# espnet/espnet

Hardware: AMD Instinct MI355X
Metric: audio-seconds/sec (RTF^-1), Conformer-ASR, 10 s utterances (higher is better)
Workload: dtype bf16; 1 GPU; BASELINE.json configs[1]: Conformer-small (12x256d, 4 heads), HIP STFT/log-mel + HIP encoder + greedy CTC (G1) + hypotheses collated to the host, 32 x 10 s utterances per GPU per step, V=5000; batch_per_gpu=32, global_batch=32, parallelism=utterance-dp1

## Files before the change

### espnet_amd/asr/encoder/conformer_encoder.py

```python
import ctypes as C
import math
import os
import threading
import weakref
from typing import List, Optional, Tuple

import torch

from espnet_amd import lib as L
from espnet_amd.nets_utils import (SUBSAMPLING_CONVS, SUBSAMPLING_MIN_FRAMES, conv2d_subsampled_lengths,
                                   conv_out_size)
from espnet_amd.packing import PackedModule

_POS_PROJ_LOCK = threading.Lock()
_ENC_CALL_LOCK = threading.Lock()
_TLS = threading.local()

LN_EPS = 1e-12


class LayerNorm(torch.nn.LayerNorm):
    def __init__(self, nout):
        super().__init__(nout, eps=LN_EPS)

# ... 58 lines not shown
        self.norm_ff_macaron = LayerNorm(size)
        self.norm_conv = LayerNorm(size)
        self.norm_final = LayerNorm(size)


def _fused_enabled(enc) -> bool:
    import os

    return bool(getattr(enc, "fused", True)) and os.environ.get("ESPNET_AMD_FUSED", "1") != "0"


def pack_k_units(w: torch.Tensor) -> torch.Tensor:
    n, k = w.shape
    assert k == 256 and n % 64 == 0, (n, k)
    return w.detach().reshape(n // 64, 4, 16, 8, 4, 8).permute(0, 1, 3, 4, 2, 5).contiguous().reshape(n, k)


def _pad_chunks(ff: int) -> int:
    assert ff % 64 == 0, ff
    return (ff + 127) // 128 * 128


def pack_w1(w: torch.Tensor) -> torch.Tensor:
    ff = w.shape[0]
    return pack_k_units(torch.nn.functional.pad(w.detach(), (0, 0, 0, _pad_chunks(ff) - ff)))


def pack_w2(w: torch.Tensor) -> torch.Tensor:
    d, ff = w.shape
    assert d == 256 and ff % 64 == 0, (d, ff)
# ... 209 lines not shown
                wqkv=A(torch.cat([sa.linear_q.weight, sa.linear_k.weight, sa.linear_v.weight], 0)),
                bqkv=F(torch.cat([sa.linear_q.bias, sa.linear_k.bias, sa.linear_v.bias], 0)),
                pos_u=F(sa.pos_bias_u), pos_v=F(sa.pos_bias_v),
                wout=A(sa.linear_out.weight), bout=F(sa.linear_out.bias),
                pw1=A(cm.pointwise_conv1.weight.reshape(2 * d, d)[glu_perm]),
                pw1_b=F(cm.pointwise_conv1.bias[glu_perm]),
                dw_w=F(dw_w.t()), dw_b=F(dw_b),
                pw2=A(cm.pointwise_conv2.weight.reshape(d, d)), pw2_b=F(cm.pointwise_conv2.bias),
                ff_w1=A(l.feed_forward.w_1.weight), ff_b1=F(l.feed_forward.w_1.bias),
                ff_w2=A(l.feed_forward.w_2.weight), ff_b2=F(l.feed_forward.w_2.bias),
            )
            pk.fill(layers[i], lt)
        if self._fusable():
            self._pack_fused(pk, layers)
            self._pack_fused_ctc(pk, w)
        elif self.em_dtype == L.EM_BF16 and d == 512 and ff % 128 == 0 and ff >= 256 and _fused_enabled(self):
            for i, l in enumerate(self.encoders):
                lt = dict(ffm_w1p=A(pack_ffn_rows_w1(l.feed_forward_macaron.w_1.weight)),
                          ffm_w2p=A(pack_ffn_rows_w2(l.feed_forward_macaron.w_2.weight)),
                          ff_w1p=A(pack_ffn_rows_w1(l.feed_forward.w_1.weight)),
                          ff_w2p=A(pack_ffn_rows_w2(l.feed_forward.w_2.weight)),
                          pw2p=A(pack_rows_proj(l.conv_module.pointwise_conv2.weight.reshape(d, d))),
                          woutp=A(pack_rows_proj(l.self_attn.linear_out.weight)),
                          pw1f=A(pack_rows_glu(l.conv_module.pointwise_conv1.weight.reshape(2 * d, d))),
                          fp_c=F(l.conv_module.pointwise_conv1.bias[glu_chunk_order(d)]))
                if self.heads * 64 == d:
                    sa = l.self_attn
                    lt["wqkvp"] = A(pack_ffn_rows_w1(torch.cat([sa.linear_q.weight, sa.linear_k.weight, sa.linear_v.weight], 0)))
                pk.fill(layers[i], lt)
            self._pack_rows_ctc(pk, w)
# ... 267 lines not shown
```

### espnet_amd/csrc/api.hip

```cpp
#include <stdlib.h>

#include <atomic>
#include <mutex>

#include "em_common.h"
#include "switches.h"

namespace {
EmSwitches read_switches() {
  auto on = [](const char* n) { return getenv(n) != nullptr; };
  auto num = [](const char* n, int dflt) { const char* e = getenv(n); return e ? atoi(e) : dflt; };
  EmSwitches s = {};
  s.attn2_stamps = on("EM_ATTN2_STAMPS"); s.block_stamps = on("EM_BLOCK_STAMPS"); s.ffn_stamps = on("EM_FFN_STAMPS");
  s.sub2_stamps = on("EM_SUB2_STAMPS");
  s.block_no_helpers = on("ESPNET_AMD_BLOCK_NO_HELPERS");
  s.sa_split = num("ESPNET_AMD_SA_SPLIT", 0); s.sa_group = num("ESPNET_AMD_SA_GROUP", 0);
  s.no_sa_tree = on("ESPNET_AMD_NO_SA_TREE"); s.sa_tree_min_rows = num("ESPNET_AMD_SA_TREE_MIN_ROWS", 200);
  s.no_attn2_large = on("ESPNET_AMD_NO_ATTN2_LARGE"); s.no_ffn_rows = on("ESPNET_AMD_NO_FFN_ROWS");
  s.no_rows_ctc = on("ESPNET_AMD_NO_ROWS_CTC"); s.frontend_v1 = on("ESPNET_AMD_FRONTEND_V1");
  s.gemm_stages = num("ESPNET_AMD_GEMM_STAGES", 0); s.gemm_bm = num("ESPNET_AMD_GEMM_BM", 0); s.no_mid_gemm = on("ESPNET_AMD_NO_MID_GEMM");
  s.mid_tile = num("ESPNET_AMD_MID_TILE", 0); s.lng_rt = num("ESPNET_AMD_LNG_RT", 0); s.lng_wide = num("ESPNET_AMD_LNG_WIDE", 256);
  s.no_src_lnq = on("ESPNET_AMD_NO_SRC_LNQ"); s.no_tail_fusion = on("ESPNET_AMD_NO_TAIL_FUSION");
  s.stream_no_fused = on("ESPNET_AMD_STREAM_NO_FUSED"); s.stream_mha_v1 = on("ESPNET_AMD_STREAM_MHA_V1");
  s.stream_no_ctx_fold = on("ESPNET_AMD_STREAM_NO_CTX_FOLD"); s.stream_no_ln_gemm = on("ESPNET_AMD_STREAM_NO_LN_GEMM");
  s.stream_fused_min = num("ESPNET_AMD_STREAM_FUSED_MIN", 1); s.no_sub12 = on("ESPNET_AMD_NO_SUB12");
  s.stream_ffn_split = num("ESPNET_AMD_STREAM_FFN_SPLIT", 0); s.stream_split_att = on("ESPNET_AMD_STREAM_SPLIT_ATT");
  s.dec_ffn_split = num("ESPNET_AMD_DEC_FFN_SPLIT", 0); s.dec_ffn_rows = num("ESPNET_AMD_DEC_FFN_ROWS", 0); s.no_rows_qkv = on("ESPNET_AMD_NO_ROWS_QKV"); s.ffn_rows_min_fill = num("ESPNET_AMD_FFN_ROWS_MIN_FILL", 0);
  return s;
}
std::atomic<const EmSwitches*> g_sw{nullptr};
std::mutex g_sw_mu;
}

const EmSwitches& em_sw() {
  const EmSwitches* p = g_sw.load(std::memory_order_acquire);
  if (!p) {
    std::lock_guard<std::mutex> lk(g_sw_mu);
    p = g_sw.load(std::memory_order_acquire);
    if (!p) {
      p = new EmSwitches(read_switches());
// ... 49 lines not shown
```

### espnet_amd/csrc/block.hip

```cpp
#include <stdio.h>
#include <stdlib.h>

#include <type_traits>

#include "em_common.h"
#include "switches.h"

namespace {

constexpr int D = 256;
constexpr int BM = 32;
constexpr int NT = 256;
constexpr int NC = 256;
constexpr int UNIT = 32768;
constexpr int PAR_FLOATS = EM_BLOCK_PARAM_GROUP;
constexpr int PAR_BYTES = PAR_FLOATS * 4;
constexpr int MAX_GROUPS = 4;
constexpr int PAR_OFF = 0;
constexpr int RED_OFF = PAR_OFF + MAX_GROUPS * PAR_BYTES;
constexpr int TOUCH_OFF = RED_OFF + 2048;
constexpr int TILE_OFF = TOUCH_OFF + 1024;
constexpr int ABUF_OFF = TILE_OFF + 32768;
constexpr int WK_OFF = ABUF_OFF + 16384;
constexpr int XCH_OFF = WK_OFF + 32768;
constexpr int XSLOT = 8192;
constexpr int SMEM_BYTES = XCH_OFF + 49152;
static_assert(ABUF_OFF % 1024 == 0 && TILE_OFF % 1024 == 0 && SMEM_BYTES <= 160 * 1024, "LDS layout");
constexpr int KW_MAX = 31, TROWS_MAX = BM + KW_MAX - 1;
constexpr int TPITCH = 528;
static_assert(TROWS_MAX * TPITCH <= 32768, "conv tile");
constexpr int CPAR_OFF = XCH_OFF;
constexpr int ABUF64_OFF = XCH_OFF + 8192;
static_assert(PAR_BYTES <= 8192 && ABUF64_OFF + 32768 <= SMEM_BYTES, "fold layout");

typedef const __attribute__((address_space(1))) unsigned char* GU8;
typedef const __attribute__((address_space(1))) bf16x8* GFRAG;
constexpr int BAR_UNIT = 1, BAR_PARAMS = 2, BAR_TILE = 4, BAR_LAST = 8;

#ifndef EM_BLOCK_DBG
#define EM_BLOCK_DBG 0
#endif

#ifndef EM_BLOCK_VAR
#define EM_BLOCK_VAR 0
#endif
#ifndef EM_BLOCK_FINE
#define EM_BLOCK_FINE 0
#endif
// ... 32 lines not shown
      if (ff_b1g) ff_b1g += sidx * nch_s * 64;
    }
  }
  bool ffn_exit = false;
  constexpr int KW = KWT, HALF = KWT / 2, TROWS = BM + KWT - 1;
  static_assert(KWT == 31 || KWT == 15, "depthwise conv width");
  constexpr int dbg = EM_BLOCK_DBG;
  using MM = Mma<bf16>;
  constexpr bool HAS_C = (MODE & EM_BLOCK_C) != 0, HAS_D = (MODE & EM_BLOCK_D) != 0;
  constexpr bool HAS_A = (MODE & EM_BLOCK_A) != 0, FINAL = (MODE & EM_BLOCK_FINAL) != 0;
  constexpr bool CTC = (MODE & EM_BLOCK_CTC) != 0;
  constexpr bool FOLD = HAS_C && HAS_D;
  constexpr bool ATT = (MODE & EM_BLOCK_ATT) != 0;
  static_assert(!ATT || (HAS_C && !HAS_D && !HAS_A && !FINAL), "block<ATT|C> is the only instantiation with the attention phase");
  static_assert(!FOLD || KWT == 31, "the folded C part is written for the 15-frame halo of k = 31");
  extern __shared__ __attribute__((aligned(1024))) unsigned char smem[];
  unsigned char* const abuf = smem + ABUF_OFF;
  float* const red0 = (float*)(smem + RED_OFF);
  float* const par = (float*)(smem + PAR_OFF);

  const int tid = threadIdx.x, lane = tid & 63;
  const int wave = __builtin_amdgcn_readfirstlane(tid >> 6);
  const int nf = wave & 3;
  const int lr = lane & 15, lg = lane >> 4;
  int b = blockIdx.y, t0 = blockIdx.x * BM;
  const int T = a.T;
  if constexpr (ATT) {
    const int gx = gridDim.x, lid = blockIdx.y * gx + blockIdx.x, grp = lid / (8 * gx);
    if ((int)blockIdx.y < a.B && grp * 8 + 8 <= a.B) {
      b = grp * 8 + (lid & 7);
// ... 196 lines not shown
    }
  };
  constexpr int MAXT = 16;
  auto touch = [&]() __attribute__((always_inline)) {
#ifdef EM_BLOCK_NO_TOUCH
    return;
#endif
    const int nwg = gridDim.x * gridDim.y;
    const int per_xcc = (nwg + 7) >> 3;
    const int nworker = per_xcc * 4;
    const int worker = (int)((blockIdx.y * gridDim.x + blockIdx.x) >> 3) * 4 + wave;
    const unsigned dst = TOUCH_OFF + wave * 256;
    const int loff = lane * 128;
    int total = (HAS_C ? 48 : 0) + (HAS_D ? 16 + 8 * nch : 0) + (HAS_A ? 48 + 8 * nch : 0);
    if (CTC) total += a.ctc_units * 4;
#pragma unroll 1
    for (int i = 0; i < MAXT && worker + i * nworker < total; ++i) {
      int j = worker + i * nworker;
      const unsigned char* p = nullptr;
      auto take = [&](const void* base, int n) __attribute__((always_inline)) {
        if (p == nullptr) {
          if (j < n) p = (const unsigned char*)base + (size_t)j * 8192;
          else j -= n;
        }
      };
      if (HAS_C) {
        take(a.wout, 16);
        take(a.pw1f, 32);
      }
      if (HAS_D) {
        take(a.pw2, 16);
        take(ff_w1, nch * 4);
        take(ff_w2, nch * 4);
      }
      if (HAS_A) {
        take(ffm_w1, nch * 4);
        take(ffm_w2, nch * 4);
        take(a.wqkv, 48);
      }
      if (CTC) take(a.ctc_w, a.ctc_units * 4);
// ... 1119 lines not shown
    }
    if constexpr (!HAS_A && !FINAL) {
      store_x();
      if (a.last_dst) {
        float* const dst = a.last_dst + (size_t)b * a.row_stride;
#pragma unroll
        for (int mi = 0; mi < 2; ++mi)
          if (t0 + mi * 16 + lr == T - 1) {
#pragma unroll
            for (int f = 0; f < 4; ++f) *(float4*)(dst + 64 * f + ncol) = xr[mi][f];
          }
      }
      touch_done();
      return;
    }
  } else {
    const bool ctx_slot = a.row0_src != nullptr && t0 == 0 && lr == 0;
    const float* const s0 = ctx_slot ? a.row0_src + (size_t)b * a.row_stride : a.x + mrow[0] * D;
#pragma unroll
    for (int f = 0; f < 4; ++f) xr[0][f] = *(const float4*)(s0 + 64 * f + ncol);
#pragma unroll
    for (int f = 0; f < 4; ++f) xr[1][f] = *(const float4*)(a.x + mrow[1] * D + 64 * f + ncol);
  }

  if (HAS_A) {
    stamp(30);
    const float* const pa0 = HAS_D ? pb2 : pb0;
    const float* const pa1 = HAS_D ? pb3 : pb1;
    if constexpr (HAS_D) {
      ln_to_act(pa0, 0, 256, 0);
    } else {
      touch();
      ln_to_act_pre(pa0, 0, 256, 0,
                    [&] { read_unit(ffm_w1, 0, ring[0]); read_unit(ffm_w1, 1, ring[1]); read_w2(ffm_w2, 0, 0, ring[2]); }, std::integral_constant<int, 24>{},
                    [&] { read_w2(ffm_w2, 0, 1, ring[3]); }, std::integral_constant<int, 8>{});
    }
    stamp(15);
    ffn(pa0, 512, 1536, 0.5f, ffm_w1, ffm_w2, true, ffm_b1g, a.wqkv, [&] { read_unit(a.wqkv, 2, ring[2]); });
    if constexpr (RELU) {
      if (ffn_exit) return;
    }
    stamp(22);
    ln_to_act(pa1, 0, 256, 0);
    stamp(15);
    const int H = D / 64;
    stream_k(a.wqkv, std::integral_constant<int, 12>{}, [&](const WF& cur, int u) {
      const int which = u >> 2, head = u & 3;
// ... 126 lines not shown
extern "C" int em_conformer_block_fused(int mode, const EmBlockArgs* a, void* stream) {
  if (!a || !a->x || !a->params || a->B <= 0 || a->T <= 0) return EM_ERR_BAD_ARG;
  const bool relu = (mode & EM_BLOCK_RELU) != 0;
  mode &= ~EM_BLOCK_RELU;
  if (a->d != D || a->ff <= 0 || a->ff % 64 != 0 || a->ff > 4096) return EM_ERR_UNSUPPORTED;
  hipStream_t s = (hipStream_t)stream;
  const bool need_a = (mode & EM_BLOCK_A) != 0, need_d = (mode & EM_BLOCK_D) != 0;
  if (!relu && a->ff > 1024 && (need_a || need_d)) return EM_ERR_UNSUPPORTED;
  if (relu && ((need_a && !a->ffm_b1g) || (need_d && !a->ff_b1g))) return EM_ERR_BAD_ARG;
  if (relu && mode != EM_BLOCK_A && mode != EM_BLOCK_D && mode != (EM_BLOCK_ATT | EM_BLOCK_C)) return EM_ERR_UNSUPPORTED;
  if (a->ffn_split > 1 && (need_a || need_d)) {
    const int nch_all = ((a->ff >> 6) + 1) & ~1;
    if (!relu || a->ffn_split > 16 || nch_all % (2 * a->ffn_split) != 0 || !a->ffn_part || !a->ffn_ticket) return EM_ERR_BAD_ARG;
  }
  if (!relu && mode == EM_BLOCK_D) return EM_ERR_UNSUPPORTED;
  if (need_a) {
    if (!a->ffm_w1 || !a->ffm_w2 || !a->wqkv || !a->qh || !a->kh || !a->vt) return EM_ERR_BAD_ARG;
    if (a->Tpad % 64 != 0 || a->Tpad < em_cdiv(a->T, BM) * BM) return EM_ERR_BAD_ARG;
  }
  if (need_d) {
    if ((!a->glu && !(mode & EM_BLOCK_C)) || !a->pw2 || !a->ff_w1 || !a->ff_w2 || !a->dw_w || !a->dw_b) return EM_ERR_BAD_ARG;
    if (a->kernel != (relu ? 15 : 31)) return EM_ERR_UNSUPPORTED;
  }
  if (mode == EM_BLOCK_C && (!a->ctx || !a->glu || !a->wout || !a->pw1f)) return EM_ERR_BAD_ARG;
  if (mode & EM_BLOCK_ATT) {
    if (mode != (EM_BLOCK_ATT | EM_BLOCK_C)) return EM_ERR_UNSUPPORTED;
    if (!a->glu || !a->wout || !a->pw1f || !a->qh || !a->kh || !a->vt) return EM_ERR_BAD_ARG;
    if (a->Tpad % 64 != 0 || a->Tpad < em_cdiv(a->T, BM) * BM) return EM_ERR_BAD_ARG;
    if (relu) {
      if (a->T > 64 || a->kv_frag) return EM_ERR_UNSUPPORTED;
// ... 5 lines not shown
    if (!a->ctx || !a->wout || !a->pw1f || !a->params_c) return EM_ERR_BAD_ARG;
    if (need_a && (!a->x_out || a->x_out == a->x)) return EM_ERR_BAD_ARG;
  }
  if ((mode & EM_BLOCK_FINAL) && (!a->enc_out || !a->enc_act)) return EM_ERR_BAD_ARG;
  if (mode & EM_BLOCK_CTC) {
    if ((mode & ~EM_BLOCK_C) != (EM_BLOCK_D | EM_BLOCK_FINAL | EM_BLOCK_CTC) || !a->ctc_w || !a->ctc_b || !a->ctc_ids) return EM_ERR_BAD_ARG;
    if (a->ctc_units <= 0) return EM_ERR_BAD_ARG;
  }
  const double M = (double)a->B * a->T;
  double flops = 0.0;
  if (mode & EM_BLOCK_C) flops += 2.0 * M * D * (D + 2 * D);
  if (mode & EM_BLOCK_ATT) flops += 6.0 * a->B * 4 * (double)a->T * a->T * 64;
  if (mode & EM_BLOCK_D) flops += 2.0 * M * D * (D + 2.0 * a->ff);
  if (mode & EM_BLOCK_A) flops += 2.0 * M * D * (2.0 * a->ff + 3 * D);
  if (mode & EM_BLOCK_CTC) flops += 2.0 * M * D * 64.0 * a->ctc_units;
  const bool rec = em_prof_begin(stream);
  int rc = EM_ERR_BAD_ARG;
  if (relu) {
    if (mode == EM_BLOCK_A) rc = launch_block<EM_BLOCK_A, 31, true>(a, s);
    else if (mode == (EM_BLOCK_ATT | EM_BLOCK_C)) rc = launch_block<EM_BLOCK_ATT | EM_BLOCK_C, 31, true>(a, s);
    else rc = launch_block<EM_BLOCK_D, 15, true>(a, s);
    if (rec) em_prof_end(stream, flops, EM_PROF_BLOCK);
    return rc;
  }
  switch (mode) {
    case EM_BLOCK_C: rc = launch_block<EM_BLOCK_C>(a, s); break;
    case EM_BLOCK_ATT | EM_BLOCK_C: rc = launch_block<EM_BLOCK_ATT | EM_BLOCK_C>(a, s); break;
    case EM_BLOCK_A: rc = launch_block<EM_BLOCK_A>(a, s); break;
    case EM_BLOCK_D | EM_BLOCK_A: rc = launch_block<EM_BLOCK_D | EM_BLOCK_A>(a, s); break;
    case EM_BLOCK_D | EM_BLOCK_FINAL: rc = launch_block<EM_BLOCK_D | EM_BLOCK_FINAL>(a, s); break;
    case EM_BLOCK_D | EM_BLOCK_FINAL | EM_BLOCK_CTC:
      rc = launch_block<EM_BLOCK_D | EM_BLOCK_FINAL | EM_BLOCK_CTC>(a, s);
      break;
    case EM_BLOCK_C | EM_BLOCK_D | EM_BLOCK_A: rc = launch_block<EM_BLOCK_C | EM_BLOCK_D | EM_BLOCK_A>(a, s); break;
    case EM_BLOCK_C | EM_BLOCK_D | EM_BLOCK_FINAL: rc = launch_block<EM_BLOCK_C | EM_BLOCK_D | EM_BLOCK_FINAL>(a, s); break;
    case EM_BLOCK_C | EM_BLOCK_D | EM_BLOCK_FINAL | EM_BLOCK_CTC:
      rc = launch_block<EM_BLOCK_C | EM_BLOCK_D | EM_BLOCK_FINAL | EM_BLOCK_CTC>(a, s);
      break;
  }
  if (rec) em_prof_end(stream, flops, EM_PROF_BLOCK);
  return rc;
}
```

### espnet_amd/csrc/encoder.hip

```cpp
#include <math.h>
#include <stdlib.h>

#include "em_common.h"
#include "switches.h"
#include "subsample.h"

namespace {

constexpr float LN_EPS = 1e-12f;

inline size_t align_up(size_t v) { return (v + 255) & ~(size_t)255; }

struct Ws {
  size_t c1, c2, c3, x, xn, big, g, g2, ctx, pall, qh, kh, vt, ppk, total;
  int Tpad;
};
inline int fused_tpad(int T) { return (T + 255) / 256 * 256; }
inline Ws layout(int dtype, const EmConformerWeights* w, int B, int T_f) {
  const size_t es = dtype == EM_BF16 ? 2 : 4;
  em_sub::Geo g;
  em_sub::geo(w->subsample, T_f, w->n_mels, &g);
  const size_t M = (size_t)B * g.T_out, d = w->d;
  size_t mb[3];
  em_sub::map_bytes(g, B, w->d, es, mb);
// ... 72 lines not shown
  r.ctc = r.ffn && !no_rows_ctc && w->ctc_ids && w->ctc_w && w->ctc_b && w->ctc_units > 0;
  return r;
}

inline int encode_plan(int dtype, const EmConformerWeights* w, int flags, long M = 0) {
  if (rows_plan(dtype, w, flags, M).ctc) return EM_ENC_PLAN_CTC_IDS;
  const int d = w->d, h = w->heads, ff = w->ff, L = w->num_blocks;
  const EmConformerLayer* ly = w->layers;
  bool fused = dtype == EM_BF16 && d == 256 && h == 4 && ff <= 1024 && w->kernel == 31 && !w->legacy_relpos &&
               !(flags & EM_ENC_NO_FUSED) && ly && L > 0 && ly[0].fp_a != nullptr;
  for (int l = 0; fused && l < L; ++l)
    fused = ly[l].pw1f && ly[l].fp_c && ly[l].fp_da && ly[l].ffm_w2p && ly[l].ff_w2p && ly[l].woutp && ly[l].pw2p &&
            ly[l].ff_w1p && ly[l].ffm_w1p && ly[l].wqkvp;
  if (!fused) return 0;
  const bool ctc = w->ctc_ids && w->ctc_w && w->ctc_b && w->ctc_units > 0;
  return EM_ENC_PLAN_FUSED | (ctc ? EM_ENC_PLAN_CTC_IDS : 0);
}

#define EM_TRY(expr)            \
  do {                          \
    int rc__ = (expr);          \
    if (rc__ != EM_OK) return rc__; \
  } while (0)

}

extern "C" size_t em_conformer_workspace_bytes(int dtype, const EmConformerWeights* w, int32_t B,
                                               int32_t T_f) {
  if (!w || B <= 0 || T_f < em_sub::min_frames(w->subsample)) return 0;
  return layout(dtype, w, B, T_f).total;
}
// ... 29 lines not shown
  if (!em_sub::geo(w->subsample, T_f, w->n_mels, &g)) return EM_ERR_UNSUPPORTED;
  const int T = g.T_out, M = B * T;
  unsigned char* ws = (unsigned char*)workspace;
  void* c1 = ws + s.c1;
  void* c2 = ws + s.c2;
  void* c3 = ws + s.c3;
  float* x = (float*)(ws + s.x);
  void* xn = ws + s.xn;
  void* big = ws + s.big;
  void* gl = ws + s.g;
  void* g2 = ws + s.g2;
  void* ctx = ws + s.ctx;
  void* pall = ws + s.pall;
  const size_t es = dtype == EM_BF16 ? 2 : 4;

  EM_TRY(em_sub::run(dtype, w, g, feats, mvn_partial, flens, B, c1, c2, c3, x, stream, w->conv1_wf, w->conv2_wf));
  const EmConformerLayer* ly = w->layers;
  if (flags & EM_ENC_POS_PROJECTED)
    pall = const_cast<void*>(pos_emb);
  else
    EM_TRY(gemm(dtype, EM_EPI_STORE, pos_emb, w->wpos_all, pall, nullptr, w->legacy_relpos ? T : 2 * T - 1, L * d, d, d,
                L * d, 1.f, stream));
  const int plan = encode_plan(dtype, w, flags);
  const bool fused = (plan & EM_ENC_PLAN_FUSED) != 0;
  if (fused) {
    void* qh = ws + s.qh;
    void* kh = ws + s.kh;
    void* vt = ws + s.vt;
    if (32 * em_cdiv(T, 32) < s.Tpad &&
        hipMemsetAsync(vt, 0, (size_t)B * d * s.Tpad * es, (hipStream_t)stream) != hipSuccess)
      return EM_ERR_LAUNCH;
    EmBlockArgs ba = {};
    ba.B = B; ba.T = T; ba.Tpad = s.Tpad; ba.d = d; ba.ff = ff; ba.kernel = w->kernel; ba.eps = LN_EPS;
    ba.x = x; ba.ctx = ctx; ba.glu = gl; ba.qh = qh; ba.kh = kh; ba.vt = vt;
    ba.enc_out = enc_out; ba.enc_act = enc_act; ba.tlens = conv_lens;
    auto set_a = [&](const EmConformerLayer& q) { ba.ffm_w1 = q.ffm_w1p; ba.ffm_w2 = q.ffm_w2p; ba.wqkv = q.wqkvp; };
    const bool att_c = !(flags & EM_ENC_FOLD_C) && !(flags & EM_ENC_SPLIT_ATT);
    void* ppk = ws + s.ppk;
    const int npg = em_relpos_pos_fragments(T);
    if (att_c) {
      if ((flags & EM_ENC_POS_PROJECTED) && (flags & EM_ENC_POS_PACKED))
        ppk = (unsigned char*)const_cast<void*>(pos_emb) + align_up((size_t)(2 * T - 1) * L * d * es);
      else
        EM_TRY(em_relpos_pack_pos_bf16(pall, L * d, T, L, ppk, stream));
      ba.kv_frag = 1;
    }
    set_a(ly[0]);
    ba.params = ly[0].fp_a;
    EM_TRY(em_conformer_block_fused(EM_BLOCK_A, &ba, stream));
    const bool no_fold = !(flags & EM_ENC_FOLD_C);
    const int cbit = no_fold ? 0 : EM_BLOCK_C;
    float* xa = x;
    float* xb = (float*)big;
    for (int l = 0; l < L; ++l) {
      const EmConformerLayer& q = ly[l];
      ba.wout = q.woutp; ba.pw1f = q.pw1f;
      if (att_c) {
        ba.pos = (const unsigned char*)ppk + (size_t)l * 4 * npg * 2048; ba.ldp = npg; ba.pos_u = q.pos_u; ba.pos_v = q.pos_v;
        ba.klens = olens; ba.params = q.fp_c;
        EM_TRY(em_conformer_block_fused(EM_BLOCK_ATT | EM_BLOCK_C, &ba, stream));
      } else {
        EM_TRY(em_relpos_attention2_bf16(qh, kh, vt, (const unsigned char*)pall + (size_t)l * d * es, L * d, q.pos_u,
                                         q.pos_v, olens, B, T, s.Tpad, h, ctx, stream));
      }
// ... 143 lines not shown
```

### espnet_amd/csrc/subsample.h

```cpp
#pragma once
#include "switches.h"
#include <math.h>
#include <stdlib.h>

#include "em_common.h"

namespace em_sub {

struct Geo {
  int n;
  int T[4], F[4];
  int k[3], s[3];
  int T_out, F_out;
};

inline int mode_of(int subsample) { return subsample == 0 ? 4 : subsample; }

inline int min_frames(int subsample) {
  switch (mode_of(subsample)) {
    case 6: return 11;
    case 8: return 15;
    default: return 7;
  }
}
// ... 12 lines not shown
    g->F[i + 1] = (g->F[i] - g->k[i]) / g->s[i] + 1;
    if (g->T[i] < g->k[i] || g->F[i] < g->k[i]) return false;
  }
  g->T_out = g->T[convs];
  g->F_out = g->F[convs];
  return g->T_out >= 1 && g->F_out >= 1;
}

inline void map_bytes(const Geo& g, int B, int d, size_t es, size_t out[3]) {
  for (int i = 0; i < 3; ++i) out[i] = i <= g.n ? (size_t)B * g.T[i + 1] * g.F[i + 1] * d * es : 0;
}

template <typename W>
inline int run(int dtype, const W* w, const Geo& g, const float* feats, const float* mvn_partial,
               const int32_t* flens, int B, void* c1, void* c2, void* c3, float* x, void* stream,
               const void* conv1_wf = nullptr, const void* conv2_wf = nullptr) {
  const int d = w->d;
  int rc = EM_ERR_UNSUPPORTED;
  const bool no_fused = em_sw().no_sub12;
  const bool try_fused = dtype == EM_BF16 && conv1_wf && conv2_wf && mode_of(w->subsample) == 4 && !no_fused;
  if (try_fused)
    rc = em_conv2d_sub12_bf16(feats, mvn_partial, flens, B, g.T[0], g.F[0], conv1_wf, conv2_wf, w->conv2_b, d, c2, stream);
  if (rc != EM_OK && rc != EM_ERR_UNSUPPORTED) return rc;
  const bool fused = rc == EM_OK;
  if (!fused) {
    rc = em_conv2d_sub1(dtype, feats, mvn_partial, flens, B, g.T[0], g.F[0], w->conv1_w, w->conv1_b, d, c1, stream);
    if (rc != EM_OK) return rc;
  }
  const void* in = fused ? c2 : c1;
  void* outs[2] = {c2, c3};
  const void* ws[2] = {w->conv2_w, w->conv3_w};
  const float* bs[2] = {w->conv2_b, w->conv3_b};
  for (int i = fused ? 1 : 0; i < g.n; ++i) {
    EmGemmArgs a = {};
    a.A = in; a.W = ws[i]; a.C = outs[i]; a.bias = bs[i];
    a.M = B * g.T[i + 2] * g.F[i + 2]; a.N = d; a.K = g.k[i + 1] * g.k[i + 1] * d; a.lda = 0; a.ldc = d; a.scale = 1.f;
    a.T1 = g.T[i + 1]; a.F1 = g.F[i + 1]; a.T2 = g.T[i + 2]; a.F2 = g.F[i + 2]; a.d = d;
    a.conv_k = g.k[i + 1]; a.conv_s = g.s[i + 1];
    if (!a.W || !a.C) return EM_ERR_BAD_ARG;
    rc = em_gemm(dtype, EM_EPI_RELU, EM_A_CONV2, &a, stream);
    if (rc != EM_OK) return rc;
    in = outs[i];
  }
  EmGemmArgs e = {};
  e.A = in; e.W = w->embed_w; e.C = x; e.bias = w->embed_b;
  e.M = B * g.T_out; e.N = d; e.K = g.F_out * d; e.lda = g.F_out * d; e.ldc = d; e.scale = sqrtf((float)d);
  return em_gemm(dtype, EM_EPI_SCALE_F32, EM_A_PLAIN, &e, stream);
}

}
```

### espnet_amd/csrc/switches.h

```cpp
#pragma once

struct EmSwitches {
  bool attn2_stamps, block_stamps, ffn_stamps, sub2_stamps;
  bool block_no_helpers;
  int sa_split, sa_group;
  bool no_sa_tree;
  int sa_tree_min_rows;
  bool no_rows_qkv;
  bool no_attn2_large, no_ffn_rows, no_rows_ctc;
  bool frontend_v1;
  int gemm_stages, gemm_bm;
  bool no_mid_gemm;
  int mid_tile, lng_rt, lng_wide;
  bool no_src_lnq, no_tail_fusion;
  bool stream_no_fused, stream_mha_v1, stream_no_ctx_fold, stream_no_ln_gemm;
  int stream_fused_min;
  bool stream_split_att;
  int stream_ffn_split;
  bool no_sub12;
  int ffn_rows_min_fill;
  int dec_ffn_rows;
  int dec_ffn_split;
};

const EmSwitches& em_sw();
```

### espnet_amd/lib.py

```python
import ctypes as C
import os
from pathlib import Path

_LIB_PATH = Path(__file__).resolve().parent / "lib" / "libespnet_amd.so"

EM_OK = 0
EM_LNF_RELU_FRAG, EM_LNF_STORE, EM_LNF_STORE_F32 = 0, 1, 2
EM_ERR_UNSUPPORTED, EM_ERR_BAD_ARG, EM_ERR_TOO_SHORT, EM_ERR_LAUNCH, EM_ERR_WORKSPACE, EM_ERR_IO = -1, -2, -3, -4, -5, -6
EM_F32, EM_BF16 = 0, 1
(EM_EPI_STORE, EM_EPI_SWISH, EM_EPI_RELU, EM_EPI_RESID_F32, EM_EPI_SCALE_F32, EM_EPI_GLU,
 EM_EPI_STORE_F32, _EM_EPI_UNUSED_7, _EM_EPI_UNUSED_8, EM_EPI_ARGMAX_PART, EM_EPI_GELU, EM_EPI_QK_HEADS,
 EM_EPI_VT_HEADS) = range(13)
EM_A_PLAIN, EM_A_CONV2 = 0, 1

EM_DW_SWISH, EM_DW_LINEAR, EM_DW_GATE, EM_DW_SELFRES = range(4)
EM_ENC_ISOLATE_UTTS = 1
EM_ENC_NO_FUSED = 2
EM_ENC_POS_PROJECTED = 4
EM_ENC_FOLD_C = 8
EM_ENC_SPLIT_ATT = 16
EM_ENC_POS_PACKED = 32


def EM_ENC_IN_FLIGHT(n):
    return (int(n) & 15) << 8


EM_ENC_PLAN_FUSED, EM_ENC_PLAN_CTC_IDS = 1, 2
EM_BLOCK_C, EM_BLOCK_D, EM_BLOCK_A, EM_BLOCK_FINAL, EM_BLOCK_CTC, EM_BLOCK_RELU, EM_BLOCK_ATT = 1, 2, 4, 8, 16, 32, 64
EM_BLOCK_PARAM_GROUP = 1792
EM_BLOCK_CTC_MAX_UNITS = 88
EM_PROF_GEMM, EM_PROF_BLOCK, EM_PROF_ATTN, EM_PROF_ROWS = 0, 1, 2, 3
DTYPES = {"float32": EM_F32, "fp32": EM_F32, "f32": EM_F32, "bfloat16": EM_BF16, "bf16": EM_BF16}


class TooShortUttError(Exception):

    def __init__(self, message, actual_size, limit, indices=None):
        super().__init__(message)
        self.actual_size = actual_size
        self.limit = limit
        self.indices = indices


# ... 16 lines not shown
               "ff_b2", "pw1f", "ffm_w2p", "ff_w2p", "woutp", "pw2p", "ff_w1p", "ffm_w1p", "wqkvp", "fp_c", "fp_da", "fp_a"]


class EmConformerLayer(C.Structure):
    _fields_ = [(n, C.c_void_p) for n in _LAYER_PTRS]


class EmBlockArgs(C.Structure):
    _fields_ = [(n, C.c_int32) for n in ("B", "T", "Tpad", "d", "ff", "kernel")] + [("eps", C.c_float)] + \
               [(n, C.c_void_p) for n in ("x", "ctx", "glu", "qh", "kh", "vt", "enc_out", "enc_act", "tlens", "wout",
                                          "pw1f", "pw2", "ff_w1", "ff_w2", "dw_w", "dw_b", "ffm_w1", "ffm_w2", "wqkv",
                                          "params", "ctc_w", "ctc_b", "ctc_ids")] + [("ctc_units", C.c_int32)] + \
               [("x_out", C.c_void_p), ("params_c", C.c_void_p), ("ffm_b1g", C.c_void_p), ("ff_b1g", C.c_void_p),
                ("row0_src", C.c_void_p), ("last_dst", C.c_void_p), ("row_stride", C.c_int32), ("ldp", C.c_int32),
                ("pos", C.c_void_p), ("pos_u", C.c_void_p), ("pos_v", C.c_void_p), ("klens", C.c_void_p), ("kv_frag", C.c_int32),
                ("ffn_split", C.c_int32), ("ffn_part", C.c_void_p), ("ffn_ticket", C.c_void_p), ("att_mask", C.c_int32)]


EM_ROWS_FFN, EM_ROWS_GLU = 0, 1
EM_ROWS_ACT_SWISH, EM_ROWS_ACT_RELU = 0, 1


class EmFfnRowsArgs(C.Structure):
    _fields_ = [(n, C.c_void_p) for n in ("xn_in", "x", "w1p", "w2p", "b1", "b2", "g1", "be1", "g2", "be2", "xn_out",
                                          "out_f32")] + \
               [(n, C.c_int32) for n in ("M", "d", "ff", "ln_mode")] + [("scale", C.c_float), ("eps", C.c_float)] + \
               [(n, C.c_void_p) for n in ("pre_in", "pre_w", "pre_b", "pre_g", "pre_be")] + [("main", C.c_int32)] + \
               [(n, C.c_void_p) for n in ("post_w", "post_b", "post_ids")] + [("post_chunks", C.c_int32), ("post_vocab", C.c_int32)] + \
               [(n, C.c_void_p) for n in ("post_q", "post_k", "post_vt")] + [("post_T", C.c_int32), ("post_Tpad", C.c_int32)] + \
               [("act", C.c_int32)]


class EmConformerWeights(C.Structure):
    _fields_ = [("d", C.c_int32), ("heads", C.c_int32), ("ff", C.c_int32),
                ("num_blocks", C.c_int32), ("kernel", C.c_int32), ("n_mels", C.c_int32),
                ("conv1_w", C.c_void_p), ("conv1_b", C.c_void_p), ("conv2_w", C.c_void_p),
                ("conv2_b", C.c_void_p), ("embed_w", C.c_void_p), ("embed_b", C.c_void_p),
                ("wpos_all", C.c_void_p), ("after_norm_g", C.c_void_p),
                ("after_norm_b", C.c_void_p), ("layers", C.POINTER(EmConformerLayer)),
                ("subsample", C.c_int32), ("conv3_w", C.c_void_p), ("conv3_b", C.c_void_p),
                ("legacy_relpos", C.c_int32), ("ctc_w", C.c_void_p), ("ctc_b", C.c_void_p),
                ("ctc_ids", C.c_void_p), ("ctc_units", C.c_int32), ("conv1_wf", C.c_void_p), ("conv2_wf", C.c_void_p)]


_EBF_LAYER_PTRS = ["norm_ff_mac_g", "norm_ff_mac_b", "norm_mha_g", "norm_mha_b", "norm_mlp_g", "norm_mlp_b",
                   "norm_ff_g", "norm_ff_b", "norm_final_g", "norm_final_b", "ffm_w1", "ffm_w2", "ff_w1", "ff_w2",
                   "ffm_b1", "ffm_b2", "ff_b1", "ff_b2", "wqkv", "bqkv", "pos_u", "pos_v", "wout", "bout",
                   "proj1_w", "proj1_b", "csgu_norm_g", "csgu_norm_b", "csgu_conv_w", "csgu_conv_b", "proj2_w",
                   "proj2_b", "merge_conv_w", "merge_conv_b", "merge_w", "merge_b", "pool_w", "pool_b", "wproj_w",
                   "wproj_b", "ffm_w1p", "ffm_w2p", "ff_w1p", "ff_w2p", "wqkvp"]
EM_MERGE_CONCAT, EM_MERGE_LEARNED_AVE = 0, 1


class EmEBranchformerLayer(C.Structure):
    _fields_ = [(n, C.c_void_p) for n in _EBF_LAYER_PTRS]


# ... 297 lines not shown
```

### include/espnet_amd.h

```cpp
#ifndef ESPNET_AMD_H_
#define ESPNET_AMD_H_

#include <stddef.h>
#include <stdint.h>

#ifdef __cplusplus
extern "C" {
#endif

#define EM_OK 0
#define EM_ERR_UNSUPPORTED (-1)
#define EM_ERR_BAD_ARG (-2)
#define EM_ERR_TOO_SHORT (-3)
#define EM_ERR_LAUNCH (-4)
#define EM_ERR_WORKSPACE (-5)
#define EM_ERR_IO (-6)

#define EM_F32 0
#define EM_BF16 1

#define EM_EPI_STORE 0
#define EM_EPI_SWISH 1
#define EM_EPI_RELU 2
#define EM_EPI_RESID_F32 3
// ... 133 lines not shown
  const void* embed_w;
  const float* embed_b;
  const void* wpos_all;
  const float *after_norm_g, *after_norm_b;
  const EmConformerLayer* layers;
  int32_t subsample;
  const void* conv3_w;
  const float* conv3_b;
  int32_t legacy_relpos;
  const void* ctc_w;
  const float* ctc_b;
  int32_t* ctc_ids;
  int32_t ctc_units;
  const void* conv1_wf;
  const void* conv2_wf;
} EmConformerWeights;

#define EM_ENC_ISOLATE_UTTS 1
#define EM_ENC_NO_FUSED 2
#define EM_ENC_FOLD_C 8
#define EM_ENC_SPLIT_ATT 16
#define EM_ENC_POS_PACKED 32
#define EM_ENC_POS_PROJECTED 4
#define EM_ENC_IN_FLIGHT(n) (((n) & 15) << 8)

#define EM_ENC_PLAN_FUSED 1
#define EM_ENC_PLAN_CTC_IDS 2
int em_conformer_encode_plan(int dtype, const EmConformerWeights* w, int32_t flags);
int em_conformer_encode_plan_for(int dtype, const EmConformerWeights* w, int32_t flags, int32_t B, int32_t T_f);

size_t em_conformer_workspace_bytes(int dtype, const EmConformerWeights* w, int32_t B, int32_t T_f);

int em_conformer_encode(int dtype, const EmConformerWeights* w, const float* feats,
                        const float* mvn_partial, const int32_t* flens, const int32_t* olens,
                        int32_t B, int32_t T_f, const void* pos_emb, void* workspace,
                        size_t workspace_bytes, float* enc_out, void* enc_act, int32_t flags,
                        void* stream);

#define EM_BLOCK_C 1
#define EM_BLOCK_D 2
#define EM_BLOCK_A 4
#define EM_BLOCK_FINAL 8
#define EM_BLOCK_CTC 16
#define EM_BLOCK_RELU 32
#define EM_BLOCK_ATT 64
#define EM_BLOCK_PARAM_GROUP 1792
typedef struct EmBlockArgs {
  int32_t B, T, Tpad, d, ff, kernel;
  float eps;
  float* x;
  const void* ctx;
  void* glu;
  void *qh, *kh, *vt;
  float* enc_out;
  void* enc_act;
  const int32_t* tlens;
  const void *wout, *pw1f;
  const void *pw2, *ff_w1, *ff_w2;
  const float *dw_w, *dw_b;
  const void *ffm_w1, *ffm_w2, *wqkv;
// ... 6 lines not shown
  const float* params_c;
  const float* ffm_b1g;
  const float* ff_b1g;
  const float* row0_src;
  float* last_dst;
  int32_t row_stride;
  int32_t ldp;
  const void* pos;
  const float *pos_u, *pos_v;
  const int32_t* klens;
  int32_t kv_frag;
  int32_t ffn_split;
  float* ffn_part;
  int32_t* ffn_ticket;
  int32_t att_mask;
} EmBlockArgs;
int em_conformer_block_fused(int mode, const EmBlockArgs* args, void* stream);
int em_relpos_pos_fragments(int32_t T);
int em_relpos_pack_pos_bf16(const void* pall, int32_t ldp, int32_t T, int32_t L, void* out, void* stream);

typedef struct EmFfnRowsArgs {
  const void* xn_in;
  float* x;
  const void *w1p, *w2p;
  const float *b1, *b2;
  const float *g1, *be1, *g2, *be2;
  void* xn_out;
  float* out_f32;
  int32_t M, d, ff, ln_mode;
  float scale, eps;
// ... 410 lines not shown
```

Baseline: 356,800 audio-s/s.

## Fold conv2d-subsampling embed linear into first fused conformer block

```diff
diff --git a/espnet_amd/asr/encoder/conformer_encoder.py b/espnet_amd/asr/encoder/conformer_encoder.py
--- a/espnet_amd/asr/encoder/conformer_encoder.py
+++ b/espnet_amd/asr/encoder/conformer_encoder.py
@@ -96,6 +96,20 @@
     n, k = w.shape
     assert k == 256 and n % 64 == 0, (n, k)
     return w.detach().reshape(n // 64, 4, 16, 8, 4, 8).permute(0, 1, 3, 4, 2, 5).contiguous().reshape(n, k)
+
+
+def pack_embed_units(weight: torch.Tensor, d: int = 256) -> torch.Tensor:
+    n, k = weight.shape
+    assert n == d == 256 and k % d == 0 and k >= d, (n, k, d)
+    wf = weight.detach().reshape(d, d, k // d).permute(2, 0, 1)
+    return torch.cat([pack_k_units(wf[f]) for f in range(k // d)], dim=0)
+
+
+def unpack_embed_units(units: torch.Tensor, d: int = 256) -> torch.Tensor:
+    f2 = units.shape[0] // d
+    assert units.shape == (f2 * d, d) and d == 256, units.shape
+    wf = units.reshape(f2 * d // 64, 4, 8, 4, 16, 8).permute(0, 1, 4, 2, 3, 5).reshape(f2, d, d)
+    return wf.permute(1, 2, 0).reshape(d, d * f2)
 
 
 def _pad_chunks(ff: int) -> int:
@@ -335,6 +349,8 @@
         if self._fusable():
             self._pack_fused(pk, layers)
             self._pack_fused_ctc(pk, w)
+            if getattr(self, "input_layer", "conv2d") == "conv2d":
+                pk.fill(w, dict(embed_wu=A(pack_embed_units(e.out.weight, d))))
         elif self.em_dtype == L.EM_BF16 and d == 512 and ff % 128 == 0 and ff >= 256 and _fused_enabled(self):
             for i, l in enumerate(self.encoders):
                 lt = dict(ffm_w1p=A(pack_ffn_rows_w1(l.feed_forward_macaron.w_1.weight)),
diff --git a/espnet_amd/csrc/api.hip b/espnet_amd/csrc/api.hip
--- a/espnet_amd/csrc/api.hip
+++ b/espnet_amd/csrc/api.hip
@@ -24,6 +24,7 @@
   s.stream_no_fused = on("ESPNET_AMD_STREAM_NO_FUSED"); s.stream_mha_v1 = on("ESPNET_AMD_STREAM_MHA_V1");
   s.stream_no_ctx_fold = on("ESPNET_AMD_STREAM_NO_CTX_FOLD"); s.stream_no_ln_gemm = on("ESPNET_AMD_STREAM_NO_LN_GEMM");
   s.stream_fused_min = num("ESPNET_AMD_STREAM_FUSED_MIN", 1); s.no_sub12 = on("ESPNET_AMD_NO_SUB12");
+  s.no_embed_fold = on("ESPNET_AMD_NO_EMBED_FOLD");
   s.stream_ffn_split = num("ESPNET_AMD_STREAM_FFN_SPLIT", 0); s.stream_split_att = on("ESPNET_AMD_STREAM_SPLIT_ATT");
   s.dec_ffn_split = num("ESPNET_AMD_DEC_FFN_SPLIT", 0); s.dec_ffn_rows = num("ESPNET_AMD_DEC_FFN_ROWS", 0); s.no_rows_qkv = on("ESPNET_AMD_NO_ROWS_QKV"); s.ffn_rows_min_fill = num("ESPNET_AMD_FFN_ROWS_MIN_FILL", 0);
   return s;
diff --git a/espnet_amd/csrc/block.hip b/espnet_amd/csrc/block.hip
--- a/espnet_amd/csrc/block.hip
+++ b/espnet_amd/csrc/block.hip
@@ -32,6 +32,8 @@
 constexpr int CPAR_OFF = XCH_OFF;
 constexpr int ABUF64_OFF = XCH_OFF + 8192;
 static_assert(PAR_BYTES <= 8192 && ABUF64_OFF + 32768 <= SMEM_BYTES, "fold layout");
+constexpr int EMB_G = 4, EMB_NS = 2 * EMB_G, EMB_TILE = 16384;
+static_assert((EMB_G & (EMB_G - 1)) == 0 && TILE_OFF + EMB_NS * EMB_TILE <= SMEM_BYTES, "embed tile ring");
 
 typedef const __attribute__((address_space(1))) unsigned char* GU8;
 typedef const __attribute__((address_space(1))) bf16x8* GFRAG;
@@ -94,6 +96,8 @@
   constexpr bool ATT = (MODE & EM_BLOCK_ATT) != 0;
   static_assert(!ATT || (HAS_C && !HAS_D && !HAS_A && !FINAL), "block<ATT|C> is the only instantiation with the attention phase");
   static_assert(!FOLD || KWT == 31, "the folded C part is written for the 15-frame halo of k = 31");
+  constexpr bool EMBED = (MODE & EM_BLOCK_EMBED) != 0;
+  static_assert(!EMBED || (HAS_A && !HAS_C && !HAS_D && !FINAL && !RELU), "block<EMBED|A> is the only instantiation with the embed stage");
   extern __shared__ __attribute__((aligned(1024))) unsigned char smem[];
   unsigned char* const abuf = smem + ABUF_OFF;
   float* const red0 = (float*)(smem + RED_OFF);
@@ -320,6 +324,7 @@
     const int loff = lane * 128;
     int total = (HAS_C ? 48 : 0) + (HAS_D ? 16 + 8 * nch : 0) + (HAS_A ? 48 + 8 * nch : 0);
     if (CTC) total += a.ctc_units * 4;
+    if (EMBED) total += a.embed_f2 * 16;
 #pragma unroll 1
     for (int i = 0; i < MAXT && worker + i * nworker < total; ++i) {
       int j = worker + i * nworker;
@@ -330,6 +335,7 @@
           else j -= n;
         }
       };
+      if (EMBED) take(a.embed_wu, a.embed_f2 * 16);
       if (HAS_C) {
         take(a.wout, 16);
         take(a.pw1f, 32);
@@ -1479,6 +1485,91 @@
       touch_done();
       return;
     }
+  } else if constexpr (EMBED) {
+    constexpr int G = EMB_G, NS = EMB_NS;
+    const int F2 = a.embed_f2, NU = 4 * F2;
+    const unsigned char* const c2wg = (const unsigned char*)a.embed_c2 + ((size_t)b * T + t0) * F2 * 512;
+    unsigned evoff;
+    {
+      const int r = 8 * wave + (lane >> 3), t = t0 + r;
+      evoff = (unsigned)((t < T ? r : T - 1 - t0) * F2 * 512 + (((lane & 7) ^ (lane >> 3)) << 4));
+    }
+    auto dma_tile = [&](int bin, int slot) __attribute__((always_inline)) {
+#pragma unroll
+      for (int i = 0; i < 4; ++i) {
+        const unsigned char* p = em_uniform_ptr(c2wg + (size_t)bin * 512 + i * 128);
+        const unsigned dst = __builtin_amdgcn_readfirstlane(TILE_OFF + slot * EMB_TILE + (4 * i + wave) * 1024);
+        unsigned keep;
+        asm volatile(
+            "s_mov_b32 %0, m0\n\t"
+            "s_mov_b32 m0, %3\n\t"
+            "s_nop 0\n\t"
+            "global_load_lds_dwordx4 %1, %2\n\t"
+            "s_mov_b32 m0, %0"
+            : "=&s"(keep)
+            : "v"(evoff), "s"(p), "s"(dst)
+            : "memory");
+      }
+    };
+    auto dma_group = [&](int first) __attribute__((always_inline)) {
+#pragma unroll
+      for (int j = 0; j < G; ++j)
+        if (first + j < F2) dma_tile(first + j, (first + j) & (NS - 1));
+    };
+    dma_group(0);
+    float4 eb[4];
+#pragma unroll
+    for (int f = 0; f < 4; ++f) eb[f] = *(const float4*)(a.embed_b + 64 * f + ncol);
+    k_pre(a.embed_wu, NU);
+    stamp(70);
+#pragma unroll
+    for (int mi = 0; mi < 2; ++mi)
+#pragma unroll
+      for (int f = 0; f < 4; ++f) xr[mi][f] = make_float4(0.f, 0.f, 0.f, 0.f);
+    asm volatile("s_waitcnt vmcnt(24)" ::: "memory");
+    bar(0);
+    dma_group(G);
+    touch();
+    stamp(71);
+#pragma unroll 1
+    for (int f2 = 0; f2 < F2; ++f2) {
+      if ((f2 & (G - 1)) == 0 && f2 > 0) {
+        asm volatile("s_waitcnt vmcnt(24)" ::: "memory");
+        bar(0);
+        dma_group(f2 + G);
+      }
+      const unsigned char* const tb = smem + TILE_OFF + (f2 & (NS - 1)) * EMB_TILE;
+#pragma unroll
+      for (int mi = 0; mi < 2; ++mi)
+#pragma unroll
+        for (int ks = 0; ks < 8; ++ks)
+          act[mi][ks] = *(const bf16x8*)(tb + ((ks >> 1) * 32 + mi * 16 + lr) * 128 + ((((ks & 1) * 4 + lg) ^ swz) << 4));
+#pragma unroll
+      for (int f = 0; f < 4; ++f) {
+        const int un = 4 * f2 + f + 3;
+        read_unit(a.embed_wu, un < NU ? un : NU - 1, ring[(f + 3) & 3]);
+        f32x4 c[2];
+        mma_k(ring[f], false, c);
+#pragma unroll
+        for (int mi = 0; mi < 2; ++mi) {
+          xr[mi][f].x += c[mi][0];
+          xr[mi][f].y += c[mi][1];
+          xr[mi][f].z += c[mi][2];
+          xr[mi][f].w += c[mi][3];
+        }
+      }
+    }
+    const float es = a.embed_scale;
+#pragma unroll
+    for (int mi = 0; mi < 2; ++mi)
+#pragma unroll
+      for (int f = 0; f < 4; ++f) {
+        xr[mi][f].x = (xr[mi][f].x + eb[f].x) * es;
+        xr[mi][f].y = (xr[mi][f].y + eb[f].y) * es;
+        xr[mi][f].z = (xr[mi][f].z + eb[f].z) * es;
+        xr[mi][f].w = (xr[mi][f].w + eb[f].w) * es;
+      }
+    stamp(72);
   } else {
     const bool ctx_slot = a.row0_src != nullptr && t0 == 0 && lr == 0;
     const float* const s0 = ctx_slot ? a.row0_src + (size_t)b * a.row_stride : a.x + mrow[0] * D;
@@ -1495,7 +1586,7 @@
     if constexpr (HAS_D) {
       ln_to_act(pa0, 0, 256, 0);
     } else {
-      touch();
+      if constexpr (!EMBED) touch();
       ln_to_act_pre(pa0, 0, 256, 0,
                     [&] { read_unit(ffm_w1, 0, ring[0]); read_unit(ffm_w1, 1, ring[1]); read_w2(ffm_w2, 0, 0, ring[2]); }, std::integral_constant<int, 24>{},
                     [&] { read_w2(ffm_w2, 0, 1, ring[3]); }, std::integral_constant<int, 8>{});
@@ -1652,6 +1743,11 @@
     if (!relu || a->ffn_split > 16 || nch_all % (2 * a->ffn_split) != 0 || !a->ffn_part || !a->ffn_ticket) return EM_ERR_BAD_ARG;
   }
   if (!relu && mode == EM_BLOCK_D) return EM_ERR_UNSUPPORTED;
+  if (mode & EM_BLOCK_EMBED) {
+    if (relu || mode != (EM_BLOCK_EMBED | EM_BLOCK_A)) return EM_ERR_UNSUPPORTED;
+    if (!a->embed_c2 || !a->embed_wu || !a->embed_b || a->embed_f2 <= 0) return EM_ERR_BAD_ARG;
+    if ((size_t)a->embed_f2 * 512 * 32 >= ((size_t)1 << 31)) return EM_ERR_UNSUPPORTED;
+  }
   if (need_a) {
     if (!a->ffm_w1 || !a->ffm_w2 || !a->wqkv || !a->qh || !a->kh || !a->vt) return EM_ERR_BAD_ARG;
     if (a->Tpad % 64 != 0 || a->Tpad < em_cdiv(a->T, BM) * BM) return EM_ERR_BAD_ARG;
@@ -1687,6 +1783,7 @@
   if (mode & EM_BLOCK_D) flops += 2.0 * M * D * (D + 2.0 * a->ff);
   if (mode & EM_BLOCK_A) flops += 2.0 * M * D * (2.0 * a->ff + 3 * D);
   if (mode & EM_BLOCK_CTC) flops += 2.0 * M * D * 64.0 * a->ctc_units;
+  if (mode & EM_BLOCK_EMBED) flops += 2.0 * M * D * D * a->embed_f2;
   const bool rec = em_prof_begin(stream);
   int rc = EM_ERR_BAD_ARG;
   if (relu) {
@@ -1700,6 +1797,7 @@
     case EM_BLOCK_C: rc = launch_block<EM_BLOCK_C>(a, s); break;
     case EM_BLOCK_ATT | EM_BLOCK_C: rc = launch_block<EM_BLOCK_ATT | EM_BLOCK_C>(a, s); break;
     case EM_BLOCK_A: rc = launch_block<EM_BLOCK_A>(a, s); break;
+    case EM_BLOCK_EMBED | EM_BLOCK_A: rc = launch_block<EM_BLOCK_EMBED | EM_BLOCK_A>(a, s); break;
     case EM_BLOCK_D | EM_BLOCK_A: rc = launch_block<EM_BLOCK_D | EM_BLOCK_A>(a, s); break;
     case EM_BLOCK_D | EM_BLOCK_FINAL: rc = launch_block<EM_BLOCK_D | EM_BLOCK_FINAL>(a, s); break;
     case EM_BLOCK_D | EM_BLOCK_FINAL | EM_BLOCK_CTC:
diff --git a/espnet_amd/csrc/encoder.hip b/espnet_amd/csrc/encoder.hip
--- a/espnet_amd/csrc/encoder.hip
+++ b/espnet_amd/csrc/encoder.hip
@@ -110,7 +110,8 @@
             ly[l].ff_w1p && ly[l].ffm_w1p && ly[l].wqkvp;
   if (!fused) return 0;
   const bool ctc = w->ctc_ids && w->ctc_w && w->ctc_b && w->ctc_units > 0;
-  return EM_ENC_PLAN_FUSED | (ctc ? EM_ENC_PLAN_CTC_IDS : 0);
+  const bool embed = em_sub::mode_of(w->subsample) == 4 && w->embed_wu && w->embed_b && !em_sw().no_embed_fold;
+  return EM_ENC_PLAN_FUSED | (ctc ? EM_ENC_PLAN_CTC_IDS : 0) | (embed ? EM_ENC_PLAN_EMBED_FOLD : 0);
 }
 
 #define EM_TRY(expr)            \
@@ -170,14 +171,15 @@
   void* pall = ws + s.pall;
   const size_t es = dtype == EM_BF16 ? 2 : 4;
 
-  EM_TRY(em_sub::run(dtype, w, g, feats, mvn_partial, flens, B, c1, c2, c3, x, stream, w->conv1_wf, w->conv2_wf));
+  const int plan = encode_plan(dtype, w, flags);
+  const bool embed_fold = (plan & EM_ENC_PLAN_EMBED_FOLD) != 0;
+  EM_TRY(em_sub::run(dtype, w, g, feats, mvn_partial, flens, B, c1, c2, c3, x, stream, w->conv1_wf, w->conv2_wf, embed_fold));
   const EmConformerLayer* ly = w->layers;
   if (flags & EM_ENC_POS_PROJECTED)
     pall = const_cast<void*>(pos_emb);
   else
     EM_TRY(gemm(dtype, EM_EPI_STORE, pos_emb, w->wpos_all, pall, nullptr, w->legacy_relpos ? T : 2 * T - 1, L * d, d, d,
                 L * d, 1.f, stream));
-  const int plan = encode_plan(dtype, w, flags);
   const bool fused = (plan & EM_ENC_PLAN_FUSED) != 0;
   if (fused) {
     void* qh = ws + s.qh;
@@ -203,7 +205,13 @@
     }
     set_a(ly[0]);
     ba.params = ly[0].fp_a;
-    EM_TRY(em_conformer_block_fused(EM_BLOCK_A, &ba, stream));
+    if (embed_fold) {
+      ba.embed_c2 = c2; ba.embed_wu = w->embed_wu; ba.embed_b = w->embed_b; ba.embed_f2 = g.F_out;
+      ba.embed_scale = sqrtf((float)d);
+      EM_TRY(em_conformer_block_fused(EM_BLOCK_EMBED | EM_BLOCK_A, &ba, stream));
+    } else {
+      EM_TRY(em_conformer_block_fused(EM_BLOCK_A, &ba, stream));
+    }
     const bool no_fold = !(flags & EM_ENC_FOLD_C);
     const int cbit = no_fold ? 0 : EM_BLOCK_C;
     float* xa = x;
diff --git a/espnet_amd/csrc/subsample.h b/espnet_amd/csrc/subsample.h
--- a/espnet_amd/csrc/subsample.h
+++ b/espnet_amd/csrc/subsample.h
@@ -50,7 +50,7 @@
 template <typename W>
 inline int run(int dtype, const W* w, const Geo& g, const float* feats, const float* mvn_partial,
                const int32_t* flens, int B, void* c1, void* c2, void* c3, float* x, void* stream,
-               const void* conv1_wf = nullptr, const void* conv2_wf = nullptr) {
+               const void* conv1_wf = nullptr, const void* conv2_wf = nullptr, bool convs_only = false) {
   const int d = w->d;
   int rc = EM_ERR_UNSUPPORTED;
   const bool no_fused = em_sw().no_sub12;
@@ -78,6 +78,7 @@
     if (rc != EM_OK) return rc;
     in = outs[i];
   }
+  if (convs_only) return (g.n == 1 && in == c2) ? EM_OK : EM_ERR_BAD_ARG;
   EmGemmArgs e = {};
   e.A = in; e.W = w->embed_w; e.C = x; e.bias = w->embed_b;
   e.M = B * g.T_out; e.N = d; e.K = g.F_out * d; e.lda = g.F_out * d; e.ldc = d; e.scale = sqrtf((float)d);
diff --git a/espnet_amd/csrc/switches.h b/espnet_amd/csrc/switches.h
--- a/espnet_amd/csrc/switches.h
+++ b/espnet_amd/csrc/switches.h
@@ -18,6 +18,7 @@
   bool stream_split_att;
   int stream_ffn_split;
   bool no_sub12;
+  bool no_embed_fold;
   int ffn_rows_min_fill;
   int dec_ffn_rows;
   int dec_ffn_split;
diff --git a/espnet_amd/lib.py b/espnet_amd/lib.py
--- a/espnet_amd/lib.py
+++ b/espnet_amd/lib.py
@@ -26,8 +26,8 @@
     return (int(n) & 15) << 8
 
 
-EM_ENC_PLAN_FUSED, EM_ENC_PLAN_CTC_IDS = 1, 2
-EM_BLOCK_C, EM_BLOCK_D, EM_BLOCK_A, EM_BLOCK_FINAL, EM_BLOCK_CTC, EM_BLOCK_RELU, EM_BLOCK_ATT = 1, 2, 4, 8, 16, 32, 64
+EM_ENC_PLAN_FUSED, EM_ENC_PLAN_CTC_IDS, EM_ENC_PLAN_EMBED_FOLD = 1, 2, 4
+EM_BLOCK_C, EM_BLOCK_D, EM_BLOCK_A, EM_BLOCK_FINAL, EM_BLOCK_CTC, EM_BLOCK_RELU, EM_BLOCK_ATT, EM_BLOCK_EMBED = 1, 2, 4, 8, 16, 32, 64, 128
 EM_BLOCK_PARAM_GROUP = 1792
 EM_BLOCK_CTC_MAX_UNITS = 88
 EM_PROF_GEMM, EM_PROF_BLOCK, EM_PROF_ATTN, EM_PROF_ROWS = 0, 1, 2, 3
@@ -74,7 +74,9 @@
                [("x_out", C.c_void_p), ("params_c", C.c_void_p), ("ffm_b1g", C.c_void_p), ("ff_b1g", C.c_void_p),
                 ("row0_src", C.c_void_p), ("last_dst", C.c_void_p), ("row_stride", C.c_int32), ("ldp", C.c_int32),
                 ("pos", C.c_void_p), ("pos_u", C.c_void_p), ("pos_v", C.c_void_p), ("klens", C.c_void_p), ("kv_frag", C.c_int32),
-                ("ffn_split", C.c_int32), ("ffn_part", C.c_void_p), ("ffn_ticket", C.c_void_p), ("att_mask", C.c_int32)]
+                ("ffn_split", C.c_int32), ("ffn_part", C.c_void_p), ("ffn_ticket", C.c_void_p), ("att_mask", C.c_int32),
+                ("embed_c2", C.c_void_p), ("embed_wu", C.c_void_p), ("embed_b", C.c_void_p), ("embed_f2", C.c_int32),
+                ("embed_scale", C.c_float)]
 
 
 EM_ROWS_FFN, EM_ROWS_GLU = 0, 1
@@ -100,7 +102,8 @@
                 ("after_norm_b", C.c_void_p), ("layers", C.POINTER(EmConformerLayer)),
                 ("subsample", C.c_int32), ("conv3_w", C.c_void_p), ("conv3_b", C.c_void_p),
                 ("legacy_relpos", C.c_int32), ("ctc_w", C.c_void_p), ("ctc_b", C.c_void_p),
-                ("ctc_ids", C.c_void_p), ("ctc_units", C.c_int32), ("conv1_wf", C.c_void_p), ("conv2_wf", C.c_void_p)]
+                ("ctc_ids", C.c_void_p), ("ctc_units", C.c_int32), ("conv1_wf", C.c_void_p), ("conv2_wf", C.c_void_p),
+                ("embed_wu", C.c_void_p)]
 
 
 _EBF_LAYER_PTRS = ["norm_ff_mac_g", "norm_ff_mac_b", "norm_mha_g", "norm_mha_b", "norm_mlp_g", "norm_mlp_b",
diff --git a/include/espnet_amd.h b/include/espnet_amd.h
--- a/include/espnet_amd.h
+++ b/include/espnet_amd.h
@@ -171,6 +171,7 @@
   int32_t ctc_units;
   const void* conv1_wf;
   const void* conv2_wf;
+  const void* embed_wu;
 } EmConformerWeights;
 
 #define EM_ENC_ISOLATE_UTTS 1
@@ -183,6 +184,7 @@
 
 #define EM_ENC_PLAN_FUSED 1
 #define EM_ENC_PLAN_CTC_IDS 2
+#define EM_ENC_PLAN_EMBED_FOLD 4
 int em_conformer_encode_plan(int dtype, const EmConformerWeights* w, int32_t flags);
 int em_conformer_encode_plan_for(int dtype, const EmConformerWeights* w, int32_t flags, int32_t B, int32_t T_f);
 
@@ -201,6 +203,7 @@
 #define EM_BLOCK_CTC 16
 #define EM_BLOCK_RELU 32
 #define EM_BLOCK_ATT 64
+#define EM_BLOCK_EMBED 128
 #define EM_BLOCK_PARAM_GROUP 1792
 typedef struct EmBlockArgs {
   int32_t B, T, Tpad, d, ff, kernel;
@@ -237,6 +240,11 @@
   float* ffn_part;
   int32_t* ffn_ticket;
   int32_t att_mask;
+  const void* embed_c2;
+  const void* embed_wu;
+  const float* embed_b;
+  int32_t embed_f2;
+  float embed_scale;
 } EmBlockArgs;
 int em_conformer_block_fused(int mode, const EmBlockArgs* args, void* stream);
 int em_relpos_pos_fragments(int32_t T);
```

Result: no change. 354,900 audio-s/s, median of 2 (-0.6%).
